# AsherBond/0-kno-vectorx

Measured on AMD Instinct MI355X. Metric: header_range_256 proofs/sec, higher is better.
Workload: dtype u64 (Goldilocks) / u8 (hashes)

## Files before the change

0-kno-vectorx_amd/csrc/vx_fri.hip:

```cpp
#include "poseidon.cuh"
#include "vx_internal.h"

struct FoldArgs {
    const uint64_t* in;
    uint64_t* out;
    int log_n, arity_bits;
    uint64_t beta_pow[5][2];
    uint64_t sinv_half[5];
    uint64_t half;
    const uint64_t* tw_inv;
};

__device__ __forceinline__ uint64_t root_pow_inv(const uint64_t* tw, uint64_t e, int log_s) {
    uint64_t E = (e << (32 - log_s)) & 0xFFFFFFFFULL;
    uint64_t r = tw[4096 + (E >> 22)];
    if (log_s > 10) r = gl_mul(r, tw[2048 + ((E >> 11) & 2047)]);
    if (log_s > 21) r = gl_mul(r, tw[E & 2047]);
    return r;
}

template <int A>
__global__ __launch_bounds__(256) void k_fri_fold(FoldArgs a) {
    constexpr int ARITY = 1 << A;
    const size_t M = (size_t)1 << (a.log_n - A);
// ... 31 lines not shown
    const size_t M = (size_t)1 << log_m;
    size_t q = blockIdx.x * (size_t)blockDim.x + threadIdx.x;
    if (q >= M) return;
    uint64_t s[12];
#pragma unroll
    for (int k = 0; k < 12; ++k) s[k] = 0;
    if (ARITY == 1 || ARITY == 2) {
#pragma unroll
        for (int t = 0; t < ARITY; ++t) {
            const uint64_t* p = evals + 2 * (q + (size_t)brev32(t, A) * M);
            s[2 * t] = p[0];
            s[2 * t + 1] = p[1];
        }
    } else {
#pragma unroll
        for (int t0 = 0; t0 < ARITY; t0 += 4) {
#pragma unroll
            for (int t = 0; t < 4; ++t) {
                const uint64_t* p = evals + 2 * (q + (size_t)brev32(t0 + t, A) * M);
                s[2 * t] = p[0];
                s[2 * t + 1] = p[1];
            }
            poseidon_permute(s);
        }
    }
    uint64_t* d = digests + 4 * (size_t)brev32((uint32_t)q, log_m);
    d[0] = s[0];
    d[1] = s[1];
    d[2] = s[2];
    d[3] = s[3];
}
__global__ void k_fri_gather_leaves(const uint64_t* evals, int log_n, int arity_bits, const uint64_t* idx, size_t n_idx,
                                    uint64_t* out) {
    const int arity = 1 << arity_bits;
    size_t t = blockIdx.x * (size_t)blockDim.x + threadIdx.x;
    if (t >= n_idx * arity) return;
    size_t k = t >> arity_bits;
    int e = (int)(t & (arity - 1));
    const int log_m = log_n - arity_bits;
    size_t q = brev32((uint32_t)idx[k], log_m);
    const uint64_t* p = evals + 2 * (q + ((size_t)brev32(e, arity_bits) << log_m));
    out[2 * t] = p[0];
    out[2 * t + 1] = p[1];
}

__global__ __launch_bounds__(256) void k_fri_pow(const uint64_t* state12, int pos, int bits, uint64_t base, uint64_t count,
                                                 unsigned long long* best) {
    uint64_t t = blockIdx.x * (uint64_t)blockDim.x + threadIdx.x;
    uint64_t stride = (uint64_t)gridDim.x * blockDim.x;
    for (; t < count; t += stride) {
        uint64_t cand = base + t;
        if (cand >= __hip_atomic_load(best, __ATOMIC_RELAXED, __HIP_MEMORY_SCOPE_AGENT)) return;
        uint64_t s[12];
#pragma unroll
        for (int k = 0; k < 12; ++k) s[k] = state12[k];
#pragma unroll
        for (int k = 0; k < 12; ++k)
            if (k == pos) s[k] = cand;
        poseidon_permute(s);
        if (bits == 0 || (s[7] >> (64 - bits)) == 0) atomicMin(best, (unsigned long long)cand);
    }
}

extern "C" {

int32_t vx_fri_fold(vx_ctx* ctx, const vx_buf* evals, int log_n, int arity_bits, const uint64_t beta[2], uint64_t shift,
// ... 68 lines not shown
    vx_merkle_levels_launch(ctx, t->levels, M, cap);
    hipError_t le = hipGetLastError();
    if (le != hipSuccess) {
        vx_pool_free(ctx, t->levels);
        delete t;
        return vx_fail(ctx, VX_ERR_DEVICE, "fri tree launch: %s", hipGetErrorString(le));
    }
    *out = t;
    return VX_OK;
}

int32_t vx_fri_leaves_dev(vx_ctx* ctx, const uint64_t* evals, int log_n, int arity_bits, const uint64_t* leaf_idx, size_t n_idx,
                          uint64_t* out);

extern "C" {
int32_t vx_fri_layer_tree(vx_ctx* ctx, const vx_buf* evals, int log_n, int arity_bits, int cap_height, vx_tree** out) {
    if (!ctx || !evals || !out) return VX_ERR_ARG;
    VX_CHECK(arity_bits >= 0 && arity_bits <= 5 && arity_bits <= log_n && log_n <= 30, "fri tree: bad log_n %d / arity_bits %d", log_n, arity_bits);
    VX_CHECK(evals->n >= ((size_t)2 << log_n), "fri tree: evals too small");
    return vx_fri_layer_tree_dev(ctx, evals->d, log_n, arity_bits, cap_height, out);
}

int32_t vx_fri_leaves(vx_ctx* ctx, const vx_buf* evals, int log_n, int arity_bits, const uint64_t* leaf_idx, size_t n_idx,
                      uint64_t* out) {
    if (!ctx || !evals || !leaf_idx || !out) return VX_ERR_ARG;
    VX_CHECK(arity_bits >= 0 && arity_bits <= 5 && arity_bits <= log_n && log_n <= 30, "fri leaves: bad shape");
    size_t N = (size_t)1 << log_n, M = N >> arity_bits;
    VX_CHECK(evals->n >= 2 * N, "fri leaves: evals too small");
    for (size_t i = 0; i < n_idx; ++i) VX_CHECK(leaf_idx[i] < M, "fri leaves: index out of range");
    return vx_fri_leaves_dev(ctx, evals->d, log_n, arity_bits, leaf_idx, n_idx, out);
}
}

int32_t vx_fri_leaves_dev(vx_ctx* ctx, const uint64_t* evals_d, int log_n, int arity_bits, const uint64_t* leaf_idx, size_t n_idx,
                          uint64_t* out) {
    if (!n_idx) return VX_OK;
    size_t tot = n_idx << arity_bits;
    uint64_t* sc;
    VX_TRY(vx_scratch(ctx, n_idx + 2 * tot, &sc));
    VX_HIP(hipMemcpyAsync(sc, leaf_idx, n_idx * 8, hipMemcpyHostToDevice, ctx->stream));
    hipLaunchKernelGGL(k_fri_gather_leaves, dim3((unsigned)((tot + 255) / 256)), dim3(256), 0, ctx->stream, evals_d, log_n,
                       arity_bits, (const uint64_t*)sc, n_idx, sc + n_idx);
    VX_HIP(hipGetLastError());
    VX_HIP(hipMemcpyAsync(out, sc + n_idx, 2 * tot * 8, hipMemcpyDeviceToHost, ctx->stream));
    VX_HIP(hipStreamSynchronize(ctx->stream));
    return VX_OK;
}

extern "C" {
int32_t vx_fri_pow(vx_ctx* ctx, const uint64_t state[12], int pos, int bits, uint64_t* nonce) {
    if (!ctx || !state || !nonce) return VX_ERR_ARG;
    VX_CHECK(pos >= 0 && pos < 8 && bits >= 0 && bits <= 40, "fri pow: bad pos %d / bits %d", pos, bits);
    uint64_t* sc;
    VX_TRY(vx_scratch(ctx, 16, &sc));
    unsigned long long* best = (unsigned long long*)(sc + 12);
    unsigned long long init = ~0ULL, h = ~0ULL;
    VX_HIP(hipMemcpyAsync(sc, state, 12 * 8, hipMemcpyHostToDevice, ctx->stream));
    VX_HIP(hipMemcpyAsync(best, &init, 8, hipMemcpyHostToDevice, ctx->stream));
    const uint64_t limit = 1ULL << (bits + 12 > 62 ? 62 : bits + 12);
    uint64_t chunk = 1ULL << (bits + 2 < 16 ? 16 : (bits + 2 > 22 ? 22 : bits + 2));
    for (uint64_t base = 0; base < limit; base += chunk, chunk = 1ULL << 22) {
        const unsigned blocks = (unsigned)(chunk / 256 < 2048 ? chunk / 256 : 2048);
        hipLaunchKernelGGL(k_fri_pow, dim3(blocks), dim3(256), 0, ctx->stream, sc, pos, bits, base, chunk, best);
        VX_HIP(hipGetLastError());
        VX_HIP(hipMemcpyAsync(&h, best, 8, hipMemcpyDeviceToHost, ctx->stream));
        VX_HIP(hipStreamSynchronize(ctx->stream));
        if (h != ~0ULL) {
            *nonce = h;
            return VX_OK;
        }
    }
    return vx_fail(ctx, VX_ERR_POW, "fri pow: no nonce below 2^%d", bits + 12);
}
}
```

0-kno-vectorx_amd/csrc/vx_internal.h:

```cpp
#pragma once
#include <hip/hip_runtime.h>
#include <stdint.h>
#include <map>
#include <string>
#include <vector>

#pragma GCC visibility push(default)
#include "../../include/vx.h"
#pragma GCC visibility pop

namespace glh {
static const uint64_t P = 0xFFFFFFFF00000001ULL;
static inline uint64_t add(uint64_t a, uint64_t b) {
    uint64_t s = a + b;
    return (s < a || s >= P) ? s - P : s;
}
static inline uint64_t sub(uint64_t a, uint64_t b) { return a >= b ? a - b : a + (P - b); }
static inline uint64_t reduce128(unsigned __int128 x) {
    const uint64_t lo = (uint64_t)x, hi = (uint64_t)(x >> 64), hh = hi >> 32, hl = hi & 0xFFFFFFFFULL;
    uint64_t t0, t2;
    if (__builtin_sub_overflow(lo, hh, &t0)) t0 -= 0xFFFFFFFFULL;
    if (__builtin_add_overflow(t0, hl * 0xFFFFFFFFULL, &t2)) t2 += 0xFFFFFFFFULL;
    return t2 >= P ? t2 - P : t2;
}
static inline uint64_t mul(uint64_t a, uint64_t b) { return reduce128((unsigned __int128)a * b); }
static inline uint64_t pow(uint64_t a, uint64_t e) {
    uint64_t r = 1;
    while (e) {
        if (e & 1) r = mul(r, a);
        a = mul(a, a);
        e >>= 1;
    }
    return r;
}
static inline uint64_t inv(uint64_t a) { return pow(a, P - 2); }
static const uint64_t ROOT_2_32 = 1753635133440165772ULL;
static inline uint64_t root(int log_n) {
    uint64_t r = ROOT_2_32;
    for (int i = 32; i > log_n; --i) r = mul(r, r);
    return r;
}
}

struct vx_buf {
    uint64_t* d;
    size_t n;
};

struct PowTab {
    uint64_t* d;
};

struct vx_ctx {
    int device;
    hipStream_t stream;
    hipEvent_t ev0, ev1;
    std::string err;
    PowTab tw_fwd, tw_inv;
    uint64_t *w12_fwd, *w12_inv;
    std::map<uint64_t, PowTab> shift_tabs;
    std::map<int, uint64_t*> tw2;
    uint64_t* scratch;
    size_t scratch_n;
    void* pinned;
    size_t pinned_n;
    std::map<size_t, std::vector<void*>> pool_free;
    std::map<void*, size_t> pool_live;
    vx_ctx* side = nullptr;
    std::map<uint64_t, uint64_t*> periodic_cache;
};
vx_ctx* vx_side_ctx(vx_ctx* ctx);
void* vx_pool_alloc(vx_ctx* ctx, size_t bytes);
void vx_pool_free(vx_ctx* ctx, void* p);
void vx_pool_trim(vx_ctx* ctx);

// ... 2 lines not shown
    size_t n_leaves;
    int cap_height;
    size_t total;
};

int32_t vx_fail(vx_ctx* ctx, int32_t code, const char* fmt, ...);
#define VX_HIP(call)                                                                              \
    do {                                                                                          \
        hipError_t e_ = (call);                                                                   \
        if (e_ != hipSuccess)                                                                     \
            return vx_fail(ctx, e_ == hipErrorOutOfMemory ? VX_ERR_OOM : VX_ERR_DEVICE, "%s: %s", \
                           #call, hipGetErrorString(e_));                                         \
    } while (0)
#define VX_CHECK(cond, ...)                                   \
    do {                                                      \
        if (!(cond)) return vx_fail(ctx, VX_ERR_ARG, __VA_ARGS__); \
    } while (0)
#define VX_TRY(call)            \
    do {                        \
        int32_t r_ = (call);    \
        if (r_ != VX_OK) return r_; \
    } while (0)

int32_t vx_get_shift_tab(vx_ctx* ctx, uint64_t base, PowTab* out);
int32_t vx_scratch(vx_ctx* ctx, size_t n_u64, uint64_t** out);
int32_t vx_merkle_build_dev(vx_ctx* ctx, const uint64_t* data, size_t n_leaves, size_t leaf_len, int layout,
                            int cap_height, vx_tree** out);

int32_t vx_ntt_dev(vx_ctx* ctx, uint64_t* d, int log_n, size_t n_cols, size_t col_stride, int inverse, uint64_t shift, int order);
int32_t vx_lde_dev(vx_ctx* ctx, const uint64_t* src, int log_n, size_t n_cols, int rate_bits, uint64_t shift, int src_kind,
                   uint64_t* dst, uint64_t* coeffs_out);
int32_t vx_gather_rows_dev(vx_ctx* ctx, const uint64_t* lde, int log_N, size_t n_cols, const uint64_t* leaf_idx, size_t n_idx,
                           uint64_t* out);
int32_t vx_fri_fold_dev(vx_ctx* ctx, const uint64_t* evals, int log_n, int arity_bits, const uint64_t beta[2], uint64_t shift,
                        uint64_t* out);
int32_t vx_fri_layer_tree_dev(vx_ctx* ctx, const uint64_t* evals, int log_n, int arity_bits, int cap_height, vx_tree** out);
int32_t vx_fri_leaves_dev(vx_ctx* ctx, const uint64_t* evals, int log_n, int arity_bits, const uint64_t* leaf_idx, size_t n_idx,
                          uint64_t* out);

struct Tw2 {
    const uint64_t* lo;
    const uint64_t* hi;
    int lo_bits;
};
int32_t vx_get_tw2(vx_ctx* ctx, int log_s, int inverse, Tw2* out);
int32_t vx_lde_consume_dev(vx_ctx* ctx, uint64_t* values, int log_n, size_t n_cols, int rate_bits, uint64_t shift, uint64_t* dst);
struct vx_chal_hook {
    int32_t (*fn)(void* user, const uint64_t* pub, size_t n_pub, const uint64_t* cap, size_t cap_words, uint64_t* chal, size_t n_chal);
    void* user;
};
int32_t vx_stark_prove_impl(vx_ctx* ctx, int air_id, const vx_stark_config* cfg, uint64_t* trace_d, size_t trace_len, int consume_trace,
                            int log_n, const uint64_t* public_inputs, size_t n_public, uint64_t* proof_out, size_t proof_cap,
                            size_t* proof_len, const vx_chal_hook* hook = nullptr);
void vx_shared_challenges_n(const uint64_t* const* pubs, const size_t* n_pubs, const uint64_t* const* caps, size_t k, size_t cap_words, uint64_t* out, size_t n_out);
void vx_shared_challenges(const uint64_t* pub_a, size_t n_a, const uint64_t* cap_a, const uint64_t* pub_b, size_t n_b, const uint64_t* cap_b,
                          size_t cap_words, uint64_t* out, size_t n_out);
int32_t vx_stark_verify_ext(const vx_stark_config* cfg, const uint64_t* proof, size_t proof_len, int expect_air, const uint64_t* expect_public,
                            size_t n_expect_public, const uint64_t* ext_chal, const uint64_t** apub_out, int* log_n_out, char* err, size_t errlen);
bool vx_stark_proof_peek(const uint64_t* proof, size_t len, int cap_height, const uint64_t** pub, size_t* n_pub, const uint64_t** cap);
int32_t vx_lde_keep_dev(vx_ctx* ctx, const uint64_t* values, int log_n, size_t n_cols, int rate_bits, uint64_t shift, uint64_t* coef_brev,
                        uint64_t* dst);
int32_t vx_scan_cols_dev(vx_ctx* ctx, uint64_t* data, int log_n, size_t n_cols, uint64_t* totals_host);
int32_t vx_sha_tree_trace_dev(vx_ctx* ctx, const uint8_t* state_roots, const uint8_t* data_roots, size_t n_leaves, int log_tree, uint64_t* trace_d,
                              uint64_t pub_out[17]);
int32_t vx_bus_close_dev(vx_ctx* ctx, uint64_t* z_cols, int log_n, uint64_t aux_pub[2]);
int32_t vx_ed_trace_dev(vx_ctx* ctx, const uint8_t* pubkeys, const uint8_t* sigs, const uint8_t* msg, uint32_t msg_len, const uint8_t* signed_flags, size_t n_sigs,
// ... 11 lines not shown
```

0-kno-vectorx_amd/csrc/vx_ntt.hip:

```cpp
#include <stdlib.h>
#include <utility>

#include "gl.cuh"
#include "vx_internal.h"

struct PassArgs {
    const uint64_t* src;
    uint64_t* dst;
    size_t src_col_stride, dst_col_stride;
    int log_sub;
    int log_rows;
    int log_T;
    const uint64_t* w12;
    const uint64_t* tw;
    uint64_t scale;
    int expand_bits;
    int log_coeff;
    const uint64_t* shift_tab;
    const uint64_t* tw2_lo;
    const uint64_t* tw2_hi;
    int tw2_bits;
    unsigned tw2_total;
    size_t n_cols;
    size_t n_tiles;
// ... 342 lines not shown
            }
            if (lr - qA > 0) tile_twiddle(x, w12s, tid, 8, qA, lr - qA, lT);
            tile_round<1, INV>(x, qA);
#pragma unroll
            for (int e = 0; e < 16; ++e) {
                const int i = tile_iota(tid, e, 8);
                dst[base + (size_t)(i >> lT) * m + (i & (T - 1))] = x[e];
            }
        }
    }
}

#include "ntt3.cuh"

__global__ void k_bitrev_copy(const uint64_t* in, uint64_t* out, int log_n, size_t in_stride, size_t out_stride) {
    size_t n = (size_t)1 << log_n;
    const uint64_t* s = in + blockIdx.y * in_stride;
    uint64_t* d = out + blockIdx.y * out_stride;
    for (size_t i = blockIdx.x * (size_t)blockDim.x + threadIdx.x; i < n; i += (size_t)gridDim.x * blockDim.x)
        d[i] = s[brev32((uint32_t)i, log_n)];
}
__global__ void k_scale_pow(uint64_t* d, int log_n, size_t stride, const uint64_t* tab, uint64_t mulc) {
    size_t n = (size_t)1 << log_n;
    uint64_t* c = d + blockIdx.y * stride;
    for (size_t i = blockIdx.x * (size_t)blockDim.x + threadIdx.x; i < n; i += (size_t)gridDim.x * blockDim.x) {
        uint64_t v = c[i];
        if (mulc != 1) v = gl_mul(v, mulc);
        if (tab) v = gl_mul(v, tab3_pow(tab, i));
        c[i] = v;
    }
}
__global__ void k_gather_rows(const uint64_t* lde, int log_N, size_t n_cols, const uint64_t* idx, size_t n_idx,
                              uint64_t* out) {
    size_t t = blockIdx.x * (size_t)blockDim.x + threadIdx.x;
    if (t >= n_idx * n_cols) return;
    size_t k = t / n_cols, c = t - k * n_cols;
    size_t row = brev32((uint32_t)idx[k], log_N);
    out[t] = lde[(c << log_N) + row];
}

static void plan_chunks(int L, std::vector<int>& outer, int& last) {
    last = L < 12 ? L : 12;
    int rem = L - last;
    outer.clear();
    if (rem > 0) {
        int k = (rem + 7) / 8;
        for (int i = 0; i < k; ++i) outer.push_back(rem / k + (i < rem % k ? 1 : 0));
    }
}
static inline size_t lds_bytes(int lr, int lT) {
    size_t T = (size_t)1 << lT;
    return ((size_t)1 << lr) * (T > 1 ? T + 1 : 1) * 8;
}
static bool g_ntt_v1 = getenv("VX_NTT_V1") != nullptr;
static bool g_ntt_v2 = getenv("VX_NTT_V2") != nullptr;
template <int MODE, int LR>
static void launch_ntt3(vx_ctx* ctx, PassArgs& a, unsigned gx, size_t n_cols, int inverse) {
    a.n_cols = n_cols;
    constexpr int NC = n3::cols_per_block(MODE, LR);
    const dim3 grid(gx, (unsigned)((n_cols + NC - 1) / NC)), block(256);
    if constexpr (MODE == 1 && LR == 12) {
        if (a.expand_bits == 1) { hipLaunchKernelGGL((k_ntt3<1, 0, 12, 1>), grid, block, 0, ctx->stream, a); return; }
        if (a.expand_bits == 2) { hipLaunchKernelGGL((k_ntt3<1, 0, 12, 2>), grid, block, 0, ctx->stream, a); return; }
        if (a.expand_bits == 3) { hipLaunchKernelGGL((k_ntt3<1, 0, 12, 3>), grid, block, 0, ctx->stream, a); return; }
    }
    if (inverse) hipLaunchKernelGGL((k_ntt3<MODE, 1, LR>), grid, block, 0, ctx->stream, a);
// ... 148 lines not shown
    if (log_n + rate_bits == 0) {
        VX_HIP(hipMemcpyAsync(dst, co, n_cols * 8, hipMemcpyDeviceToDevice, ctx->stream));
        return VX_OK;
    }
    return ntt_dit(ctx, co, n, dst, N, log_n + rate_bits, n_cols, 0, rate_bits, st.d);
}

int32_t vx_lde_consume_dev(vx_ctx* ctx, uint64_t* values, int log_n, size_t n_cols, int rate_bits, uint64_t shift, uint64_t* dst) {
    const size_t n = (size_t)1 << log_n, N = n << rate_bits;
    PowTab st{nullptr};
    if (shift > 1) VX_TRY(vx_get_shift_tab(ctx, shift, &st));
    if (log_n > 0) VX_TRY(ntt_dif(ctx, values, n, values, n, log_n, n_cols, 1, glh::inv((uint64_t)n % glh::P)));
    if (log_n + rate_bits == 0) {
        VX_HIP(hipMemcpyAsync(dst, values, n_cols * 8, hipMemcpyDeviceToDevice, ctx->stream));
        return VX_OK;
    }
    return ntt_dit(ctx, values, n, dst, N, log_n + rate_bits, n_cols, 0, rate_bits, st.d);
}

int32_t vx_lde_keep_dev(vx_ctx* ctx, const uint64_t* values, int log_n, size_t n_cols, int rate_bits, uint64_t shift, uint64_t* coef_brev,
                        uint64_t* dst) {
    const size_t n = (size_t)1 << log_n, N = n << rate_bits;
    PowTab st{nullptr};
    if (shift > 1) VX_TRY(vx_get_shift_tab(ctx, shift, &st));
    if (log_n == 0) VX_HIP(hipMemcpyAsync(coef_brev, values, n_cols * 8, hipMemcpyDeviceToDevice, ctx->stream));
    else VX_TRY(ntt_dif(ctx, values, n, coef_brev, n, log_n, n_cols, 1, glh::inv((uint64_t)n % glh::P)));
    if (log_n + rate_bits == 0) {
        VX_HIP(hipMemcpyAsync(dst, coef_brev, n_cols * 8, hipMemcpyDeviceToDevice, ctx->stream));
        return VX_OK;
    }
    return ntt_dit(ctx, coef_brev, n, dst, N, log_n + rate_bits, n_cols, 0, rate_bits, st.d);
}

int32_t vx_gather_rows_dev(vx_ctx* ctx, const uint64_t* lde, int log_N, size_t n_cols, const uint64_t* leaf_idx, size_t n_idx,
                           uint64_t* out) {
    if (n_idx == 0) return VX_OK;
    uint64_t* sc;
    VX_TRY(vx_scratch(ctx, n_idx + n_idx * n_cols, &sc));
    VX_HIP(hipMemcpyAsync(sc, leaf_idx, n_idx * 8, hipMemcpyHostToDevice, ctx->stream));
    size_t tot = n_idx * n_cols;
    hipLaunchKernelGGL(k_gather_rows, dim3((unsigned)((tot + 255) / 256)), dim3(256), 0, ctx->stream, lde, log_N, n_cols,
                       (const uint64_t*)sc, n_idx, sc + n_idx);
    VX_HIP(hipGetLastError());
    VX_HIP(hipMemcpyAsync(out, sc + n_idx, tot * 8, hipMemcpyDeviceToHost, ctx->stream));
    VX_HIP(hipStreamSynchronize(ctx->stream));
    return VX_OK;
}

extern "C" {

int32_t vx_ntt(vx_ctx* ctx, vx_buf* buf, size_t off, int log_n, size_t n_cols, size_t col_stride, int inverse,
               uint64_t shift, int order) {
    if (!ctx || !buf) return VX_ERR_ARG;
    VX_CHECK(log_n >= 0 && log_n <= 28, "vx_ntt: log_n %d out of range [0,28]", log_n);
    VX_CHECK(col_stride >= ((size_t)1 << log_n) && n_cols >= 1 && off + (n_cols - 1) * col_stride + ((size_t)1 << log_n) <= buf->n, "vx_ntt: columns exceed the buffer");
    return vx_ntt_dev(ctx, buf->d + off, log_n, n_cols, col_stride, inverse, shift, order);
}
}

int32_t vx_ntt_dev(vx_ctx* ctx, uint64_t* d, int log_n, size_t n_cols, size_t col_stride, int inverse, uint64_t shift, int order) {
    if (!ctx || !d) return VX_ERR_ARG;
    VX_CHECK(log_n >= 0 && log_n <= 28, "vx_ntt: log_n %d out of range [0,28]", log_n);
    size_t n = (size_t)1 << log_n;
    VX_CHECK(n_cols >= 1 && n_cols <= 65535, "vx_ntt: n_cols %zu out of range", n_cols);
    VX_CHECK(shift < GL_P, "vx_ntt: shift not canonical");
    VX_CHECK(order == VX_ORDER_NATURAL || order == VX_ORDER_BITREV, "vx_ntt: bad order");
    if (log_n == 0) return VX_OK;
    const bool coset = shift > 1;
    const unsigned gx = (unsigned)((n + 255) / 256 > 1024 ? 1024 : (n + 255) / 256);
    PowTab st{nullptr};
    if (!inverse) {
        if (coset) VX_TRY(vx_get_shift_tab(ctx, shift, &st));
        if (order == VX_ORDER_BITREV) {
            if (coset) {
                hipLaunchKernelGGL(k_scale_pow, dim3(gx, (unsigned)n_cols), dim3(256), 0, ctx->stream, d, log_n, col_stride,
// ... 57 lines not shown
```

0-kno-vectorx_amd/csrc/vx_poseidon.hip:

```cpp
#include "poseidon.cuh"
#include "poseidon_air.cuh"
#include "vx_internal.h"

__global__ __launch_bounds__(256) void k_poseidon_batch(uint64_t* states, size_t n) {
    size_t i = blockIdx.x * (size_t)blockDim.x + threadIdx.x;
    if (i >= n) return;
    uint64_t s[12];
#pragma unroll
    for (int k = 0; k < 12; ++k) s[k] = states[12 * i + k];
    poseidon_permute(s);
#pragma unroll
    for (int k = 0; k < 12; ++k) states[12 * i + k] = s[k];
}

#ifndef VX_HASH_WAVES
#define VX_HASH_WAVES 6
#endif
template <int LAYOUT>
__global__ __launch_bounds__(256) __attribute__((amdgpu_waves_per_eu(VX_HASH_WAVES, 8))) void k_hash_leaves(const uint64_t* data, size_t n_leaves, int log_n, size_t leaf_len,
                                                     uint64_t* digests) {
    size_t p = blockIdx.x * (size_t)blockDim.x + threadIdx.x;
    if (p >= n_leaves) return;
    const size_t estride = LAYOUT == VX_LEAVES_ROW_MAJOR ? 1 : n_leaves;
    const uint64_t* src = LAYOUT == VX_LEAVES_ROW_MAJOR ? data + p * leaf_len : data + p;
    size_t j = LAYOUT == VX_LEAVES_COLS_BITREV ? brev32((uint32_t)p, log_n) : p;
    uint64_t s[12];
#pragma unroll
    for (int k = 0; k < 12; ++k) s[k] = 0;
    if (leaf_len <= 4) {
        for (size_t e = 0; e < leaf_len; ++e) s[e] = src[e * estride];
    } else {
        size_t e = 0;
        for (; e + 8 <= leaf_len; e += 8) {
#pragma unroll
            for (int k = 0; k < 8; ++k) s[k] = src[(e + k) * estride];
            poseidon_permute(s);
        }
        if (e < leaf_len) {
#pragma unroll
            for (int k = 0; k < 8; ++k)
                if (e + k < leaf_len) s[k] = src[(e + k) * estride];
            poseidon_permute(s);
        }
    }
    uint64_t* d = digests + 4 * j;
    d[0] = s[0];
    d[1] = s[1];
    d[2] = s[2];
    d[3] = s[3];
}

template <int LAYOUT>
__global__ __launch_bounds__(256) void k_hash_leaves_coop(const uint64_t* data, size_t n_leaves, int log_n, size_t leaf_len,
                                                          uint64_t* digests) {
    __shared__ uint64_t lds[16 * 12];
    const int l = threadIdx.x & 15, grp = threadIdx.x >> 4;
    uint64_t* g = lds + 12 * grp;
    const size_t t = blockIdx.x * (size_t)16 + grp;
    const size_t p = t < n_leaves ? t : n_leaves - 1;
    const size_t estride = LAYOUT == VX_LEAVES_ROW_MAJOR ? 1 : n_leaves;
    const uint64_t* src = LAYOUT == VX_LEAVES_ROW_MAJOR ? data + p * leaf_len : data + p;
    const size_t j = LAYOUT == VX_LEAVES_COLS_BITREV ? brev32((uint32_t)p, log_n) : p;
    uint64_t s = 0;
    if (leaf_len <= 4) {
        if ((size_t)l < leaf_len) s = src[(size_t)l * estride];
    } else {
        for (size_t e = 0; e < leaf_len; e += 8) {
            if (l < 8 && e + l < leaf_len) s = src[(e + l) * estride];
            s = poseidon_permute_coop(s, l, g);
        }
    }
    if (l < 4 && t < n_leaves) digests[4 * j + l] = s;
}
__global__ __launch_bounds__(256) void k_merkle_level_coop(const uint64_t* child, uint64_t* parent, size_t n_parent) {
    __shared__ uint64_t lds[16 * 12];
    const int l = threadIdx.x & 15, grp = threadIdx.x >> 4;
    const size_t t = blockIdx.x * (size_t)16 + grp;
    const size_t i = t < n_parent ? t : n_parent - 1;
    uint64_t s = l < 8 ? child[8 * i + l] : 0;
    s = poseidon_permute_coop(s, l, lds + 12 * grp);
    if (l < 4 && t < n_parent) parent[4 * i + l] = s;
}
constexpr size_t COOP_MAX_LEAVES = 16384;

__global__ __launch_bounds__(256) void k_merkle_level(const uint64_t* child, uint64_t* parent, size_t n_parent) {
    size_t i = blockIdx.x * (size_t)blockDim.x + threadIdx.x;
    if (i >= n_parent) return;
    uint64_t s[12];
#pragma unroll
    for (int k = 0; k < 8; ++k) s[k] = child[8 * i + k];
    s[8] = s[9] = s[10] = s[11] = 0;
    poseidon_permute(s);
    parent[4 * i] = s[0];
    parent[4 * i + 1] = s[1];
    parent[4 * i + 2] = s[2];
    parent[4 * i + 3] = s[3];
}

__global__ void k_gather_siblings(const uint64_t* levels, size_t n_leaves, int depth, const uint64_t* idx, size_t n_idx,
                                  uint64_t* out) {
    size_t t = blockIdx.x * (size_t)blockDim.x + threadIdx.x;
    if (t >= n_idx * depth) return;
    size_t k = t / depth;
    int lvl = (int)(t - k * depth);
    size_t off = 0, cur = n_leaves;
    for (int l = 0; l < lvl; ++l) {
        off += 4 * cur;
        cur >>= 1;
    }
    size_t node = (idx[k] >> lvl) ^ 1;
    for (int e = 0; e < 4; ++e) out[4 * t + e] = levels[off + 4 * node + e];
}


__global__ __launch_bounds__(256) void k_poseidon_air_trace(const uint64_t* in, size_t n_perm, uint64_t* tr) {
    const size_t p = blockIdx.x * (size_t)256 + threadIdx.x;
    if (p >= n_perm) return;
    uint64_t s[12];
#pragma unroll
    for (int i = 0; i < 12; ++i) s[i] = gl_canon(in[12 * p + i]);
    poseidon_air_walk(s, tr, 32 * n_perm, 32 * p);
}

void vx_merkle_levels_launch(vx_ctx* ctx, uint64_t* levels, size_t n_leaves, size_t cap) {
    size_t off = 0, cur = n_leaves;
    while (cur > cap) {
        const size_t np = cur >> 1;
        if (np <= COOP_MAX_LEAVES)
            hipLaunchKernelGGL(k_merkle_level_coop, dim3((unsigned)((np + 15) / 16)), dim3(256), 0, ctx->stream, levels + off, levels + off + 4 * cur, np);
        else
            hipLaunchKernelGGL(k_merkle_level, dim3((unsigned)((np + 255) / 256)), dim3(256), 0, ctx->stream, levels + off, levels + off + 4 * cur, np);
        off += 4 * cur;
        cur = np;
    }
}

int32_t vx_merkle_build_dev(vx_ctx* ctx, const uint64_t* data, size_t n_leaves, size_t leaf_len, int layout,
                            int cap_height, vx_tree** out) {
    int log_n = 0;
    while (((size_t)1 << log_n) < n_leaves) ++log_n;
    VX_CHECK(((size_t)1 << log_n) == n_leaves, "merkle: n_leaves %zu is not a power of two", n_leaves);
    VX_CHECK(cap_height >= 0 && cap_height <= log_n, "merkle: cap_height %d > log2(n_leaves) %d", cap_height, log_n);
    VX_CHECK(leaf_len >= 1, "merkle: empty leaves");
    size_t total = 0, cur = n_leaves, cap = (size_t)1 << cap_height;
    while (cur > cap) {
        total += 4 * cur;
        cur >>= 1;
    }
    total += 4 * cur;
    vx_tree* t = new vx_tree{nullptr, n_leaves, cap_height, total};
    t->levels = (uint64_t*)vx_pool_alloc(ctx, total * 8);
    if (!t->levels) {
        delete t;
        return vx_fail(ctx, VX_ERR_OOM, "merkle: cannot allocate %zu bytes", total * 8);
    }
    unsigned g = (unsigned)((n_leaves + 255) / 256);
    if (n_leaves <= COOP_MAX_LEAVES && leaf_len > 4) {
        const unsigned gc = (unsigned)((n_leaves + 15) / 16);
        if (layout == VX_LEAVES_ROW_MAJOR)
            hipLaunchKernelGGL(k_hash_leaves_coop<VX_LEAVES_ROW_MAJOR>, dim3(gc), dim3(256), 0, ctx->stream, data, n_leaves, log_n, leaf_len, t->levels);
        else if (layout == VX_LEAVES_COLS_BITREV)
            hipLaunchKernelGGL(k_hash_leaves_coop<VX_LEAVES_COLS_BITREV>, dim3(gc), dim3(256), 0, ctx->stream, data, n_leaves, log_n, leaf_len, t->levels);
        else
            hipLaunchKernelGGL(k_hash_leaves_coop<VX_LEAVES_COLS>, dim3(gc), dim3(256), 0, ctx->stream, data, n_leaves, log_n, leaf_len, t->levels);
    } else if (layout == VX_LEAVES_ROW_MAJOR)
        hipLaunchKernelGGL(k_hash_leaves<VX_LEAVES_ROW_MAJOR>, dim3(g), dim3(256), 0, ctx->stream, data, n_leaves, log_n, leaf_len, t->levels);
    else if (layout == VX_LEAVES_COLS_BITREV)
// ... 35 lines not shown
    VX_CHECK(off + n_leaves * leaf_len <= data->n, "merkle: %zu leaves x %zu exceed the buffer", n_leaves, leaf_len);
    return vx_merkle_build_dev(ctx, data->d + off, n_leaves, leaf_len, layout, cap_height, out);
}
int32_t vx_merkle_free(vx_ctx* ctx, vx_tree* tree) {
    if (!ctx || !tree) return VX_ERR_ARG;
    vx_pool_free(ctx, tree->levels);
    delete tree;
    return VX_OK;
}
int32_t vx_merkle_cap(vx_ctx* ctx, const vx_tree* tree, uint64_t* cap_out) {
    if (!ctx || !tree || !cap_out) return VX_ERR_ARG;
    size_t cap = (size_t)4 << tree->cap_height;
    VX_HIP(hipMemcpyAsync(cap_out, tree->levels + tree->total - cap, cap * 8, hipMemcpyDeviceToHost, ctx->stream));
    VX_HIP(hipStreamSynchronize(ctx->stream));
    return VX_OK;
}
int32_t vx_merkle_leaf_digests(vx_ctx* ctx, const vx_tree* tree, uint64_t* out) {
    if (!ctx || !tree || !out) return VX_ERR_ARG;
    VX_HIP(hipMemcpyAsync(out, tree->levels, tree->n_leaves * 32, hipMemcpyDeviceToHost, ctx->stream));
    VX_HIP(hipStreamSynchronize(ctx->stream));
    return VX_OK;
}
int32_t vx_merkle_open(vx_ctx* ctx, const vx_tree* tree, const uint64_t* leaf_idx, size_t n_idx, uint64_t* siblings_out) {
    if (!ctx || !tree || !leaf_idx || !siblings_out) return VX_ERR_ARG;
    int log_n = 0;
    while (((size_t)1 << log_n) < tree->n_leaves) ++log_n;
    int depth = log_n - tree->cap_height;
    for (size_t i = 0; i < n_idx; ++i) VX_CHECK(leaf_idx[i] < tree->n_leaves, "merkle open: index out of range");
    if (depth == 0 || n_idx == 0) return VX_OK;
    uint64_t* sc;
    size_t tot = n_idx * depth;
    VX_TRY(vx_scratch(ctx, n_idx + 4 * tot, &sc));
    VX_HIP(hipMemcpyAsync(sc, leaf_idx, n_idx * 8, hipMemcpyHostToDevice, ctx->stream));
    hipLaunchKernelGGL(k_gather_siblings, dim3((unsigned)((tot + 255) / 256)), dim3(256), 0, ctx->stream, tree->levels,
                       tree->n_leaves, depth, sc, n_idx, sc + n_idx);
    VX_HIP(hipGetLastError());
    VX_HIP(hipMemcpyAsync(siblings_out, sc + n_idx, 4 * tot * 8, hipMemcpyDeviceToHost, ctx->stream));
    VX_HIP(hipStreamSynchronize(ctx->stream));
    return VX_OK;
}
}
```

0-kno-vectorx_amd/csrc/vx_stark.hip:

```cpp
#include <string.h>

#include <map>
#include <mutex>

#include <array>

#include "air_list.h"
#include "air_program.h"
#include "glh_poseidon.h"
#include "vx_internal.h"

namespace {
inline void h_poseidon(uint64_t* s) { glh::poseidon(s); }
struct Ext {
    uint64_t a, b;
};
inline Ext e_add(Ext x, Ext y) { return {glh::add(x.a, y.a), glh::add(x.b, y.b)}; }
inline Ext e_sub(Ext x, Ext y) { return {glh::sub(x.a, y.a), glh::sub(x.b, y.b)}; }
inline Ext e_mul(Ext x, Ext y) {
    return {glh::add(glh::mul(x.a, y.a), glh::mul(7, glh::mul(x.b, y.b))), glh::add(glh::mul(x.a, y.b), glh::mul(x.b, y.a))};
}
inline Ext e_scale(Ext x, uint64_t s) { return {glh::mul(x.a, s), glh::mul(x.b, s)}; }
inline Ext e_inv(Ext x) {
    uint64_t n = glh::sub(glh::mul(x.a, x.a), glh::mul(7, glh::mul(x.b, x.b)));
// ... 843 lines not shown
            const uint64_t wk = glh::pow(wi, k);
            uint64_t wcur = 1;
            for (size_t i = 0; i < fm; ++i) {
                acc = e_add(acc, e_scale(Ext{fv[2 * i], fv[2 * i + 1]}, wcur));
                wcur = glh::mul(wcur, wk);
            }
            acc = e_scale(acc, glh::mul(minv, sk));
            fc[2 * k] = acc.a;
            fc[2 * k + 1] = acc.b;
            sk = glh::mul(sk, sinv);
        }
    }
    for (size_t k = final_len; k < fm; ++k)
        VX_CHECK(fc[2 * k] == 0 && fc[2 * k + 1] == 0, "stark prove: final polynomial has degree >= %zu: the trace violates the AIR constraints", final_len);
    for (size_t k = 0; k < 2 * final_len; ++k) proof.push_back(fc[k]);
    ch.observe(fc.data(), 2 * final_len);

    {
        uint64_t st[12];
        memcpy(st, ch.st, sizeof st);
        for (int i = 0; i < ch.n_in; ++i) st[i] = ch.in[i];
        uint64_t nonce = 0;
        VX_TRY(vx_fri_pow(ctx, st, ch.n_in, cfg.pow_bits, &nonce));
        proof.push_back(nonce);
        ch.observe(nonce);
        const uint64_t resp = ch.challenge();
        VX_CHECK(cfg.pow_bits == 0 || (resp >> (64 - cfg.pow_bits)) == 0, "stark prove: PoW response check failed");
    }

    const size_t nqr = cfg.num_queries;
    std::vector<uint64_t> qidx(nqr);
    for (size_t k = 0; k < nqr; ++k) qidx[k] = ch.challenge() % N;
    const int depth0 = LN - cfg.cap_height;
    std::vector<uint64_t> rows_t(nqr * cm), rows_a(nqr * ca), rows_q(nqr * nq), sib_t(nqr * depth0 * 4), sib_a(ca ? nqr * depth0 * 4 : 0), sib_q(nqr * depth0 * 4);
    VX_TRY(vx_gather_rows_dev(ctx, trace_lde, LN, cm, qidx.data(), nqr, rows_t.data()));
    if (ca) VX_TRY(vx_gather_rows_dev(ctx, trace_lde + N * cm, LN, ca, qidx.data(), nqr, rows_a.data()));
    VX_TRY(vx_gather_rows_dev(ctx, quot_lde, LN, nq, qidx.data(), nqr, rows_q.data()));
    if (depth0 > 0) {
        VX_TRY(vx_merkle_open(ctx, t_trace, qidx.data(), nqr, sib_t.data()));
        if (ca) VX_TRY(vx_merkle_open(ctx, t_aux, qidx.data(), nqr, sib_a.data()));
        VX_TRY(vx_merkle_open(ctx, t_quot, qidx.data(), nqr, sib_q.data()));
    }
    std::vector<std::vector<uint64_t>> l_leaves(arities.size()), l_sibs(arities.size());
    std::vector<uint64_t> lidx = qidx;
    for (size_t l = 0; l < arities.size(); ++l) {
        const int a = arities[l], depth = llog[l] - a - cfg.cap_height;
        for (size_t k = 0; k < nqr; ++k) lidx[k] >>= a;
        l_leaves[l].resize(nqr * ((size_t)2 << a));
        VX_TRY(vx_fri_leaves_dev(ctx, layers[l], llog[l], a, lidx.data(), nqr, l_leaves[l].data()));
        l_sibs[l].resize(nqr * (depth > 0 ? depth : 0) * 4);
        if (depth > 0) VX_TRY(vx_merkle_open(ctx, ltrees[l], lidx.data(), nqr, l_sibs[l].data()));
    }
    for (size_t k = 0; k < nqr; ++k) {
        proof.insert(proof.end(), rows_t.begin() + k * cm, rows_t.begin() + (k + 1) * cm);
        proof.insert(proof.end(), sib_t.begin() + k * depth0 * 4, sib_t.begin() + (k + 1) * depth0 * 4);
        if (ca) {
            proof.insert(proof.end(), rows_a.begin() + k * ca, rows_a.begin() + (k + 1) * ca);
            proof.insert(proof.end(), sib_a.begin() + k * depth0 * 4, sib_a.begin() + (k + 1) * depth0 * 4);
        }
        proof.insert(proof.end(), rows_q.begin() + k * nq, rows_q.begin() + (k + 1) * nq);
        proof.insert(proof.end(), sib_q.begin() + k * depth0 * 4, sib_q.begin() + (k + 1) * depth0 * 4);
        uint64_t x_index = qidx[k];
        for (size_t l = 0; l < arities.size(); ++l) {
            const int a = arities[l], depth = llog[l] - a - cfg.cap_height;
            const size_t arity = (size_t)1 << a, within = x_index & (arity - 1);
            const uint64_t* leaf = l_leaves[l].data() + k * 2 * arity;
            for (size_t t = 0; t < arity; ++t)
                if (t != within) proof.push_back(leaf[2 * t]), proof.push_back(leaf[2 * t + 1]);
            if (depth > 0) proof.insert(proof.end(), l_sibs[l].begin() + k * depth * 4, l_sibs[l].begin() + (k + 1) * depth * 4);
            x_index >>= a;
        }
    }
    *proof_len = proof.size();
    if (!proof_out || proof_cap < proof.size()) return vx_fail(ctx, VX_ERR_BUFSZ, "stark prove: proof needs %zu words, buffer has %zu", proof.size(), proof_cap);
    memcpy(proof_out, proof.data(), proof.size() * 8);
    return VX_OK;
}
```

Baseline: 8.147.

## Batch query openings into one transfer, fuse Merkle top levels, raise tail priority

Query-phase gathers (rows, Merkle siblings, FRI leaves) are now all enqueued on one stream. They read a single uploaded index buffer, write into one scratch region, and finish with a single device-to-host copy and one sync, where before each gather did its own copy and synchronize. Separately, the small upper Merkle levels that used to launch one cooperative kernel per level are now handled by a fused k_merkle_top kernel that processes up to 9 levels per launch using LDS. The tail kernels also set a higher wave priority via s_setprio. Together these aim to cut launch and host round-trip overhead in the latency-bound tail, at the cost of more complex kernels and lower parallelism in the fused top levels.

New measurement: 8.314 (median of 6 runs). 2.1% higher.

```diff
diff --git a/0-kno-vectorx_amd/csrc/vx_fri.hip b/0-kno-vectorx_amd/csrc/vx_fri.hip
--- a/0-kno-vectorx_amd/csrc/vx_fri.hip
+++ b/0-kno-vectorx_amd/csrc/vx_fri.hip
@@ -87,6 +87,7 @@
 }
 __global__ void k_fri_gather_leaves(const uint64_t* evals, int log_n, int arity_bits, const uint64_t* idx, size_t n_idx,
                                     uint64_t* out) {
+    VX_TAIL_KERNEL_ENTRY();
     const int arity = 1 << arity_bits;
     size_t t = blockIdx.x * (size_t)blockDim.x + threadIdx.x;
     if (t >= n_idx * arity) return;
@@ -221,6 +222,12 @@
 }
 }
 
+void vx_fri_leaves_enqueue(vx_ctx* ctx, const uint64_t* evals_d, int log_n, int arity_bits, const uint64_t* idx_d, size_t n_idx, uint64_t* out_d) {
+    const size_t tot = n_idx << arity_bits;
+    if (tot == 0) return;
+    hipLaunchKernelGGL(k_fri_gather_leaves, dim3((unsigned)((tot + 255) / 256)), dim3(256), 0, ctx->stream, evals_d, log_n, arity_bits, idx_d, n_idx, out_d);
+}
+
 int32_t vx_fri_leaves_dev(vx_ctx* ctx, const uint64_t* evals_d, int log_n, int arity_bits, const uint64_t* leaf_idx, size_t n_idx,
                           uint64_t* out) {
     if (!n_idx) return VX_OK;
@@ -228,8 +235,7 @@
     uint64_t* sc;
     VX_TRY(vx_scratch(ctx, n_idx + 2 * tot, &sc));
     VX_HIP(hipMemcpyAsync(sc, leaf_idx, n_idx * 8, hipMemcpyHostToDevice, ctx->stream));
-    hipLaunchKernelGGL(k_fri_gather_leaves, dim3((unsigned)((tot + 255) / 256)), dim3(256), 0, ctx->stream, evals_d, log_n,
-                       arity_bits, (const uint64_t*)sc, n_idx, sc + n_idx);
+    vx_fri_leaves_enqueue(ctx, evals_d, log_n, arity_bits, sc, n_idx, sc + n_idx);
     VX_HIP(hipGetLastError());
     VX_HIP(hipMemcpyAsync(out, sc + n_idx, 2 * tot * 8, hipMemcpyDeviceToHost, ctx->stream));
     VX_HIP(hipStreamSynchronize(ctx->stream));
diff --git a/0-kno-vectorx_amd/csrc/vx_internal.h b/0-kno-vectorx_amd/csrc/vx_internal.h
--- a/0-kno-vectorx_amd/csrc/vx_internal.h
+++ b/0-kno-vectorx_amd/csrc/vx_internal.h
@@ -41,6 +41,15 @@
     return r;
 }
 }
+
+#ifndef VX_TAIL_PRIO
+#define VX_TAIL_PRIO 1
+#endif
+#if VX_TAIL_PRIO
+#define VX_TAIL_KERNEL_ENTRY() __builtin_amdgcn_s_setprio(3)
+#else
+#define VX_TAIL_KERNEL_ENTRY() ((void)0)
+#endif
 
 struct vx_buf {
     uint64_t* d;
@@ -109,6 +118,9 @@
                    uint64_t* dst, uint64_t* coeffs_out);
 int32_t vx_gather_rows_dev(vx_ctx* ctx, const uint64_t* lde, int log_N, size_t n_cols, const uint64_t* leaf_idx, size_t n_idx,
                            uint64_t* out);
+void vx_gather_rows_enqueue(vx_ctx* ctx, const uint64_t* lde, int log_N, size_t n_cols, const uint64_t* idx_d, size_t n_idx, uint64_t* out_d);
+void vx_merkle_open_enqueue(vx_ctx* ctx, const vx_tree* tree, const uint64_t* idx_d, size_t n_idx, uint64_t* out_d);
+void vx_fri_leaves_enqueue(vx_ctx* ctx, const uint64_t* evals, int log_n, int arity_bits, const uint64_t* idx_d, size_t n_idx, uint64_t* out_d);
 int32_t vx_fri_fold_dev(vx_ctx* ctx, const uint64_t* evals, int log_n, int arity_bits, const uint64_t beta[2], uint64_t shift,
                         uint64_t* out);
 int32_t vx_fri_layer_tree_dev(vx_ctx* ctx, const uint64_t* evals, int log_n, int arity_bits, int cap_height, vx_tree** out);
diff --git a/0-kno-vectorx_amd/csrc/vx_ntt.hip b/0-kno-vectorx_amd/csrc/vx_ntt.hip
--- a/0-kno-vectorx_amd/csrc/vx_ntt.hip
+++ b/0-kno-vectorx_amd/csrc/vx_ntt.hip
@@ -398,6 +398,7 @@
 }
 __global__ void k_gather_rows(const uint64_t* lde, int log_N, size_t n_cols, const uint64_t* idx, size_t n_idx,
                               uint64_t* out) {
+    VX_TAIL_KERNEL_ENTRY();
     size_t t = blockIdx.x * (size_t)blockDim.x + threadIdx.x;
     if (t >= n_idx * n_cols) return;
     size_t k = t / n_cols, c = t - k * n_cols;
@@ -612,6 +613,12 @@
     return ntt_dit(ctx, coef_brev, n, dst, N, log_n + rate_bits, n_cols, 0, rate_bits, st.d);
 }
 
+void vx_gather_rows_enqueue(vx_ctx* ctx, const uint64_t* lde, int log_N, size_t n_cols, const uint64_t* idx_d, size_t n_idx, uint64_t* out_d) {
+    const size_t tot = n_idx * n_cols;
+    if (tot == 0) return;
+    hipLaunchKernelGGL(k_gather_rows, dim3((unsigned)((tot + 255) / 256)), dim3(256), 0, ctx->stream, lde, log_N, n_cols, idx_d, n_idx, out_d);
+}
+
 int32_t vx_gather_rows_dev(vx_ctx* ctx, const uint64_t* lde, int log_N, size_t n_cols, const uint64_t* leaf_idx, size_t n_idx,
                            uint64_t* out) {
     if (n_idx == 0) return VX_OK;
@@ -619,8 +626,7 @@
     VX_TRY(vx_scratch(ctx, n_idx + n_idx * n_cols, &sc));
     VX_HIP(hipMemcpyAsync(sc, leaf_idx, n_idx * 8, hipMemcpyHostToDevice, ctx->stream));
     size_t tot = n_idx * n_cols;
-    hipLaunchKernelGGL(k_gather_rows, dim3((unsigned)((tot + 255) / 256)), dim3(256), 0, ctx->stream, lde, log_N, n_cols,
-                       (const uint64_t*)sc, n_idx, sc + n_idx);
+    vx_gather_rows_enqueue(ctx, lde, log_N, n_cols, sc, n_idx, sc + n_idx);
     VX_HIP(hipGetLastError());
     VX_HIP(hipMemcpyAsync(out, sc + n_idx, tot * 8, hipMemcpyDeviceToHost, ctx->stream));
     VX_HIP(hipStreamSynchronize(ctx->stream));
diff --git a/0-kno-vectorx_amd/csrc/vx_poseidon.hip b/0-kno-vectorx_amd/csrc/vx_poseidon.hip
--- a/0-kno-vectorx_amd/csrc/vx_poseidon.hip
+++ b/0-kno-vectorx_amd/csrc/vx_poseidon.hip
@@ -53,6 +53,7 @@
 template <int LAYOUT>
 __global__ __launch_bounds__(256) void k_hash_leaves_coop(const uint64_t* data, size_t n_leaves, int log_n, size_t leaf_len,
                                                           uint64_t* digests) {
+    VX_TAIL_KERNEL_ENTRY();
     __shared__ uint64_t lds[16 * 12];
     const int l = threadIdx.x & 15, grp = threadIdx.x >> 4;
     uint64_t* g = lds + 12 * grp;
@@ -72,14 +73,48 @@
     }
     if (l < 4 && t < n_leaves) digests[4 * j + l] = s;
 }
-__global__ __launch_bounds__(256) void k_merkle_level_coop(const uint64_t* child, uint64_t* parent, size_t n_parent) {
-    __shared__ uint64_t lds[16 * 12];
-    const int l = threadIdx.x & 15, grp = threadIdx.x >> 4;
-    const size_t t = blockIdx.x * (size_t)16 + grp;
-    const size_t i = t < n_parent ? t : n_parent - 1;
-    uint64_t s = l < 8 ? child[8 * i + l] : 0;
-    s = poseidon_permute_coop(s, l, lds + 12 * grp);
-    if (l < 4 && t < n_parent) parent[4 * i + l] = s;
+#ifndef VX_TOP_THREADS
+#define VX_TOP_THREADS 256
+#endif
+#ifndef VX_TOP_LANE_MIN
+#define VX_TOP_LANE_MIN 32
+#endif
+constexpr int TOP_MAX_S = 9, TOP_GROUPS = VX_TOP_THREADS / 16;
+static_assert(VX_TOP_THREADS >= (1 << (TOP_MAX_S - 1)) && VX_TOP_THREADS <= 1024, "one lane per parent of the widest level");
+__global__ __launch_bounds__(VX_TOP_THREADS) void k_merkle_top(uint64_t* levels, size_t off, size_t cur, int s) {
+    VX_TAIL_KERNEL_ENTRY();
+    __shared__ uint64_t buf[2][4 << (TOP_MAX_S - 1)];
+    __shared__ uint64_t xch[12 * TOP_GROUPS];
+    const int tid = threadIdx.x, l = tid & 15, grp = tid >> 4;
+    const uint64_t* child_g = levels + off + 4 * ((size_t)blockIdx.x << s);
+    for (int j = 1; j <= s; ++j) {
+        const int np = 1 << (s - j);
+        off += 4 * cur;
+        cur >>= 1;
+        uint64_t* parent_g = levels + off + 4 * ((size_t)blockIdx.x << (s - j));
+        uint64_t* parent_l = buf[j & 1];
+        const uint64_t* child_l = buf[(j - 1) & 1];
+        if (VX_TOP_LANE_MIN <= 256 && np >= VX_TOP_LANE_MIN) {
+            if (tid < np) {
+                uint64_t st[12];
+#pragma unroll
+                for (int k = 0; k < 8; ++k) st[k] = j == 1 ? child_g[8 * tid + k] : child_l[8 * tid + k];
+                st[8] = st[9] = st[10] = st[11] = 0;
+                poseidon_permute(st);
+#pragma unroll
+                for (int k = 0; k < 4; ++k) parent_l[4 * tid + k] = parent_g[4 * tid + k] = st[k];
+            }
+        } else {
+            for (int base = 0; base < np; base += TOP_GROUPS) {
+                const int t = base + grp, i = t < np ? t : np - 1;
+                uint64_t x = 0;
+                if (l < 8) x = j == 1 ? child_g[8 * i + l] : child_l[8 * i + l];
+                x = poseidon_permute_coop(x, l, xch + 12 * grp);
+                if (l < 4 && t < np) parent_l[4 * i + l] = parent_g[4 * i + l] = x;
+            }
+        }
+        __syncthreads();
+    }
 }
 constexpr size_t COOP_MAX_LEAVES = 16384;
 
@@ -99,6 +134,7 @@
 
 __global__ void k_gather_siblings(const uint64_t* levels, size_t n_leaves, int depth, const uint64_t* idx, size_t n_idx,
                                   uint64_t* out) {
+    VX_TAIL_KERNEL_ENTRY();
     size_t t = blockIdx.x * (size_t)blockDim.x + threadIdx.x;
     if (t >= n_idx * depth) return;
     size_t k = t / depth;
@@ -124,15 +160,33 @@
 
 void vx_merkle_levels_launch(vx_ctx* ctx, uint64_t* levels, size_t n_leaves, size_t cap) {
     size_t off = 0, cur = n_leaves;
-    while (cur > cap) {
+    while (cur > cap && (cur >> 1) > COOP_MAX_LEAVES) {
         const size_t np = cur >> 1;
-        if (np <= COOP_MAX_LEAVES)
-            hipLaunchKernelGGL(k_merkle_level_coop, dim3((unsigned)((np + 15) / 16)), dim3(256), 0, ctx->stream, levels + off, levels + off + 4 * cur, np);
-        else
-            hipLaunchKernelGGL(k_merkle_level, dim3((unsigned)((np + 255) / 256)), dim3(256), 0, ctx->stream, levels + off, levels + off + 4 * cur, np);
+        hipLaunchKernelGGL(k_merkle_level, dim3((unsigned)((np + 255) / 256)), dim3(256), 0, ctx->stream, levels + off, levels + off + 4 * cur, np);
         off += 4 * cur;
         cur = np;
     }
+    int todo = 0;
+    while ((cap << todo) < cur) ++todo;
+    while (todo > 0) {
+        const int s = todo < TOP_MAX_S ? todo : TOP_MAX_S;
+        hipLaunchKernelGGL(k_merkle_top, dim3((unsigned)(cur >> s)), dim3(VX_TOP_THREADS), 0, ctx->stream, levels, off, cur, s);
+        for (int j = 0; j < s; ++j) {
+            off += 4 * cur;
+            cur >>= 1;
+        }
+        todo -= s;
+    }
+}
+
+void vx_merkle_open_enqueue(vx_ctx* ctx, const vx_tree* tree, const uint64_t* idx_d, size_t n_idx, uint64_t* out_d) {
+    int log_n = 0;
+    while (((size_t)1 << log_n) < tree->n_leaves) ++log_n;
+    const int depth = log_n - tree->cap_height;
+    const size_t tot = n_idx * depth;
+    if (tot == 0) return;
+    hipLaunchKernelGGL(k_gather_siblings, dim3((unsigned)((tot + 255) / 256)), dim3(256), 0, ctx->stream, tree->levels,
+                       tree->n_leaves, depth, idx_d, n_idx, out_d);
 }
 
 int32_t vx_merkle_build_dev(vx_ctx* ctx, const uint64_t* data, size_t n_leaves, size_t leaf_len, int layout,
@@ -234,8 +288,7 @@
     size_t tot = n_idx * depth;
     VX_TRY(vx_scratch(ctx, n_idx + 4 * tot, &sc));
     VX_HIP(hipMemcpyAsync(sc, leaf_idx, n_idx * 8, hipMemcpyHostToDevice, ctx->stream));
-    hipLaunchKernelGGL(k_gather_siblings, dim3((unsigned)((tot + 255) / 256)), dim3(256), 0, ctx->stream, tree->levels,
-                       tree->n_leaves, depth, sc, n_idx, sc + n_idx);
+    vx_merkle_open_enqueue(ctx, tree, sc, n_idx, sc + n_idx);
     VX_HIP(hipGetLastError());
     VX_HIP(hipMemcpyAsync(siblings_out, sc + n_idx, 4 * tot * 8, hipMemcpyDeviceToHost, ctx->stream));
     VX_HIP(hipStreamSynchronize(ctx->stream));
diff --git a/0-kno-vectorx_amd/csrc/vx_stark.hip b/0-kno-vectorx_amd/csrc/vx_stark.hip
--- a/0-kno-vectorx_amd/csrc/vx_stark.hip
+++ b/0-kno-vectorx_amd/csrc/vx_stark.hip
@@ -899,42 +899,67 @@
     std::vector<uint64_t> qidx(nqr);
     for (size_t k = 0; k < nqr; ++k) qidx[k] = ch.challenge() % N;
     const int depth0 = LN - cfg.cap_height;
-    std::vector<uint64_t> rows_t(nqr * cm), rows_a(nqr * ca), rows_q(nqr * nq), sib_t(nqr * depth0 * 4), sib_a(ca ? nqr * depth0 * 4 : 0), sib_q(nqr * depth0 * 4);
-    VX_TRY(vx_gather_rows_dev(ctx, trace_lde, LN, cm, qidx.data(), nqr, rows_t.data()));
-    if (ca) VX_TRY(vx_gather_rows_dev(ctx, trace_lde + N * cm, LN, ca, qidx.data(), nqr, rows_a.data()));
-    VX_TRY(vx_gather_rows_dev(ctx, quot_lde, LN, nq, qidx.data(), nqr, rows_q.data()));
+    const size_t n_layers = arities.size();
+    std::vector<uint64_t> idx_h((1 + n_layers) * nqr);
+    std::copy(qidx.begin(), qidx.end(), idx_h.begin());
+    for (size_t l = 0; l < n_layers; ++l)
+        for (size_t k = 0; k < nqr; ++k) idx_h[(l + 1) * nqr + k] = idx_h[l * nqr + k] >> arities[l];
+    size_t words = 0;
+    auto take = [&](size_t n) {
+        const size_t at = words;
+        words += n;
+        return at;
+    };
+    const size_t sib0 = depth0 > 0 ? nqr * depth0 * 4 : 0;
+    const size_t o_rows_t = take(nqr * cm), o_rows_a = take(nqr * ca), o_rows_q = take(nqr * nq);
+    const size_t o_sib_t = take(sib0), o_sib_a = take(ca ? sib0 : 0), o_sib_q = take(sib0);
+    std::vector<size_t> o_leaves(n_layers), o_sibs(n_layers);
+    for (size_t l = 0; l < n_layers; ++l) {
+        const int a = arities[l], depth = llog[l] - a - cfg.cap_height;
+        o_leaves[l] = take(nqr * ((size_t)2 << a));
+        o_sibs[l] = take(depth > 0 ? nqr * depth * 4 : 0);
+    }
+    uint64_t* sc;
+    VX_TRY(vx_scratch(ctx, idx_h.size() + words, &sc));
+    uint64_t* const gat = sc + idx_h.size();
+    VX_HIP(hipMemcpyAsync(sc, idx_h.data(), idx_h.size() * 8, hipMemcpyHostToDevice, ctx->stream));
+    vx_gather_rows_enqueue(ctx, trace_lde, LN, cm, sc, nqr, gat + o_rows_t);
+    if (ca) vx_gather_rows_enqueue(ctx, trace_lde + N * cm, LN, ca, sc, nqr, gat + o_rows_a);
+    vx_gather_rows_enqueue(ctx, quot_lde, LN, nq, sc, nqr, gat + o_rows_q);
     if (depth0 > 0) {
-        VX_TRY(vx_merkle_open(ctx, t_trace, qidx.data(), nqr, sib_t.data()));
-        if (ca) VX_TRY(vx_merkle_open(ctx, t_aux, qidx.data(), nqr, sib_a.data()));
-        VX_TRY(vx_merkle_open(ctx, t_quot, qidx.data(), nqr, sib_q.data()));
-    }
-    std::vector<std::vector<uint64_t>> l_leaves(arities.size()), l_sibs(arities.size());
-    std::vector<uint64_t> lidx = qidx;
-    for (size_t l = 0; l < arities.size(); ++l) {
+        vx_merkle_open_enqueue(ctx, t_trace, sc, nqr, gat + o_sib_t);
+        if (ca) vx_merkle_open_enqueue(ctx, t_aux, sc, nqr, gat + o_sib_a);
+        vx_merkle_open_enqueue(ctx, t_quot, sc, nqr, gat + o_sib_q);
+    }
+    for (size_t l = 0; l < n_layers; ++l) {
         const int a = arities[l], depth = llog[l] - a - cfg.cap_height;
-        for (size_t k = 0; k < nqr; ++k) lidx[k] >>= a;
-        l_leaves[l].resize(nqr * ((size_t)2 << a));
-        VX_TRY(vx_fri_leaves_dev(ctx, layers[l], llog[l], a, lidx.data(), nqr, l_leaves[l].data()));
-        l_sibs[l].resize(nqr * (depth > 0 ? depth : 0) * 4);
-        if (depth > 0) VX_TRY(vx_merkle_open(ctx, ltrees[l], lidx.data(), nqr, l_sibs[l].data()));
-    }
+        const uint64_t* lidx_d = sc + (l + 1) * nqr;
+        vx_fri_leaves_enqueue(ctx, layers[l], llog[l], a, lidx_d, nqr, gat + o_leaves[l]);
+        if (depth > 0) vx_merkle_open_enqueue(ctx, ltrees[l], lidx_d, nqr, gat + o_sibs[l]);
+    }
+    VX_HIP(hipGetLastError());
+    std::vector<uint64_t> q(words);
+    VX_HIP(hipMemcpyAsync(q.data(), gat, words * 8, hipMemcpyDeviceToHost, ctx->stream));
+    VX_HIP(hipStreamSynchronize(ctx->stream));
+    const uint64_t *rows_t = q.data() + o_rows_t, *rows_a = q.data() + o_rows_a, *rows_q = q.data() + o_rows_q;
+    const uint64_t *sib_t = q.data() + o_sib_t, *sib_a = q.data() + o_sib_a, *sib_q = q.data() + o_sib_q;
     for (size_t k = 0; k < nqr; ++k) {
-        proof.insert(proof.end(), rows_t.begin() + k * cm, rows_t.begin() + (k + 1) * cm);
-        proof.insert(proof.end(), sib_t.begin() + k * depth0 * 4, sib_t.begin() + (k + 1) * depth0 * 4);
+        proof.insert(proof.end(), rows_t + k * cm, rows_t + (k + 1) * cm);
+        if (depth0 > 0) proof.insert(proof.end(), sib_t + k * depth0 * 4, sib_t + (k + 1) * depth0 * 4);
         if (ca) {
-            proof.insert(proof.end(), rows_a.begin() + k * ca, rows_a.begin() + (k + 1) * ca);
-            proof.insert(proof.end(), sib_a.begin() + k * depth0 * 4, sib_a.begin() + (k + 1) * depth0 * 4);
-        }
-        proof.insert(proof.end(), rows_q.begin() + k * nq, rows_q.begin() + (k + 1) * nq);
-        proof.insert(proof.end(), sib_q.begin() + k * depth0 * 4, sib_q.begin() + (k + 1) * depth0 * 4);
+            proof.insert(proof.end(), rows_a + k * ca, rows_a + (k + 1) * ca);
+            if (depth0 > 0) proof.insert(proof.end(), sib_a + k * depth0 * 4, sib_a + (k + 1) * depth0 * 4);
+        }
+        proof.insert(proof.end(), rows_q + k * nq, rows_q + (k + 1) * nq);
+        if (depth0 > 0) proof.insert(proof.end(), sib_q + k * depth0 * 4, sib_q + (k + 1) * depth0 * 4);
         uint64_t x_index = qidx[k];
-        for (size_t l = 0; l < arities.size(); ++l) {
+        for (size_t l = 0; l < n_layers; ++l) {
             const int a = arities[l], depth = llog[l] - a - cfg.cap_height;
             const size_t arity = (size_t)1 << a, within = x_index & (arity - 1);
-            const uint64_t* leaf = l_leaves[l].data() + k * 2 * arity;
+            const uint64_t* leaf = q.data() + o_leaves[l] + k * 2 * arity;
             for (size_t t = 0; t < arity; ++t)
                 if (t != within) proof.push_back(leaf[2 * t]), proof.push_back(leaf[2 * t + 1]);
-            if (depth > 0) proof.insert(proof.end(), l_sibs[l].begin() + k * depth * 4, l_sibs[l].begin() + (k + 1) * depth * 4);
+            if (depth > 0) proof.insert(proof.end(), q.data() + o_sibs[l] + k * depth * 4, q.data() + o_sibs[l] + (k + 1) * depth * 4);
             x_index >>= a;
         }
     }
```
